# chahuja/mix-stage

Hardware: AMD Instinct MI355X
Metric: train-step clips/sec (B=32, T=64, M=8) (higher is better)
Workload: dtype f32; 1 GPU; Mix-StAGE GAN train step (reference D/G coin flip, seed 4321: 457 G + 510 D steps), B=32 clips per GPU, T=64, 128-mel, 104-dim pose, M=S=8, audio branch pinned; fp32 arithmetic (the reference trains in fp64, trainer.py:138; held to it at 1e-4 pose L1); global_batch=32, parallelism=dp1, hip_graphs=True, bn_sync=local

## Files before the change

### include/mixstage_aux.h

```cpp
#ifndef MIXSTAGE_AUX_H_
#define MIXSTAGE_AUX_H_

#include "mixstage.h"

#ifdef __cplusplus
extern "C" {
#endif

int ms_set_counter_buffer(int32_t* zeroed_counters, int n);

int ms_conv_block_bwd_overlap(const ms_conv_desc* d, const float* x, const float* x2, const float* w,
                              const float* gamma, const float* running_mean, const float* running_var,
                              const float* y_raw, const float* y, const float* save, const float* dy, float* dyr,
                              float* dx, float* dx2, float* dw, float* dbias, float* dgamma, float* dbeta,
                              void* workspace, size_t workspace_bytes, void* stream, void* side_stream,
                              void* side_workspace, size_t side_workspace_bytes);

int ms_timing_enable(int on);
size_t ms_timing_report(char* buf, size_t cap);

int ms_debug_set_patch_min_workgroups(int n);
int ms_debug_set_patch_tuning(int intra_split, int force_splitk);

int ms_debug_set_conv16_tile(int wm, int wn);
int ms_debug_set_conv16_ring(int nstg, int wide8);
int ms_debug_set_wgrad16_target(int workgroups);
int ms_debug_set_wgrad16_ring(int buffers);
int ms_debug_set_wgrad_target(int workgroups);
int ms_debug_set_wgrad_wave(int on);
int ms_debug_set_conv_tile(int on);
int ms_debug_set_bn_fused(int on);
int ms_debug_set_bn_fused_min_workgroups(int n);
int ms_debug_set_skip(const char* patterns);

int ms_debug_set_clip32(int on);

int ms_debug_set_clip_corun(int on);
int ms_debug_set_clip_corun_bwd(int on);

int ms_selftest_mfma(const float* A, const float* B, float* C, int K, void* stream);
int ms_probe_peak(int kind, long iters, void* a, void* b, double* work, void* stream);

#ifdef __cplusplus
}
#endif
#endif
```

### mix_stage_amd/_lib.py

```python
import ctypes
import os

_HERE = os.path.dirname(os.path.abspath(__file__))
LIB_PATH = os.path.join(_HERE, 'libmixstage_hip.so')
_ALT_LIB = os.environ.get('MS_LIB_PATH')
if _ALT_LIB:
  LIB_PATH = _ALT_LIB

c_void_p, c_int, c_float, c_size_t = ctypes.c_void_p, ctypes.c_int, ctypes.c_float, ctypes.c_size_t


class BwdOptions(ctypes.Structure):
  _fields_ = [('side_stream', ctypes.c_void_p), ('side_workspace', ctypes.c_void_p), ('side_workspace_bytes', ctypes.c_size_t),
              ('wt_prepared', ctypes.c_void_p), ('wgrad_partials', ctypes.c_void_p), ('defer_wgrad_launch', ctypes.c_int),
              ('prev_y', ctypes.c_void_p), ('prev_y_raw', ctypes.c_void_p), ('prev_save', ctypes.c_void_p), ('prev_gamma', ctypes.c_void_p),
              ('prev_dgamma', ctypes.c_void_p), ('prev_dbeta', ctypes.c_void_p), ('prev_dbias', ctypes.c_void_p), ('prev_slope', ctypes.c_float),
              ('bn_sync', ctypes.c_void_p), ('bn_sync_words', ctypes.c_int32), ('dy_is_dyr', ctypes.c_int),
              ('dx_accum', ctypes.c_void_p)]


class LossScale(ctypes.Structure):
  _fields_ = [('scale', ctypes.c_float), ('scale_dev', ctypes.c_void_p)]


class FwdOptions(ctypes.Structure):
  _fields_ = [('w_planes', ctypes.c_void_p), ('bn_sync', ctypes.c_void_p), ('bn_sync_words', ctypes.c_int32)]


class ConvDesc(ctypes.Structure):
  _fields_ = [(n, ctypes.c_int32) for n in
              ('B', 'Cin', 'H', 'W', 'Cout', 'groups', 'KH', 'KW', 'SH', 'SW', 'PH', 'PW', 'OH', 'OW',
               'mode', 'in_mode')] + \
             [('slope', c_float), ('eps', c_float), ('momentum', c_float), ('dtype', ctypes.c_int32)]


class ChainDesc(ctypes.Structure):
  _fields_ = [(n, ctypes.c_int32) for n in ('B', 'M', 'T', 'cin0', 'C', 'P', 'n_blocks', 'mode', 'dtype', 'sync_first_word', 'keep_all_raw')] + \
             [('slope', c_float), ('eps', c_float), ('momentum', c_float)]


class ChainTensors(ctypes.Structure):
  _fields_ = [('x', ctypes.c_void_p), ('score', ctypes.c_void_p)] + \
             [(n, ctypes.c_void_p * 4) for n in ('w', 'bias', 'gamma', 'beta', 'running_mean', 'running_var', 'y_raw', 'y', 'save')] + \
             [(n, ctypes.c_void_p) for n in ('w_logits', 'bias_logits', 'z', 'soft', 'out', 'prepared', 'sync')] + \
             [('sync_words', ctypes.c_int32)]


class Prep16Item(ctypes.Structure):
  _fields_ = [('desc', ctypes.POINTER(ConvDesc))] + [(n, ctypes.c_void_p) for n in
             ('w', 'bias', 'gamma', 'beta', 'running_mean', 'running_var', 'fwd', 'dgrad')]


MS_BARE, MS_LRELU, MS_BN_TRAIN, MS_BN_EVAL = 0, 1, 2, 3
MS_DT_BN_FROZEN = 0x800
MS_IN_PLAIN, MS_IN_BCAST, MS_IN_UP2ADD = 0, 1, 2
MS_F32, MS_BF16, MS_F16, MS_DT_OUT_F32, MS_DT_BN_FOLDED = 0, 1, 2, 0x100, 0x200
MS_DT_STAT_PAIR = 0x400

_P = c_void_p
_DESC = ctypes.POINTER(ConvDesc)

SIGNATURES = {
    'ms_last_error': (ctypes.c_char_p, []),
    'ms_abi_version': (c_int, []),
    'ms_set_counter_buffer': (c_int, [_P, c_int]),
    'ms_set_bn_sync_buffer': (c_int, [_P, c_int]),
    'ms_debug_set_bn_fused': (c_int, [c_int]),
    'ms_debug_set_bn_fused_min_workgroups': (c_int, [c_int]),
    'ms_conv_block_fwd_workspace': (c_size_t, [_DESC]),
    'ms_conv_block_bwd_workspace': (c_size_t, [_DESC]),
    'ms_conv_block_fwd': (c_int, [_DESC] + [_P] * 11 + [_P, c_size_t, _P]),
    'ms_conv_block_bwd': (c_int, [_DESC] + [_P] * 17 + [_P, c_size_t, _P]),
    'ms_conv_block_bwd_overlap': (c_int, [_DESC] + [_P] * 17 + [_P, c_size_t, _P, _P, _P, c_size_t]),
    'ms_conv_block_bwd_ex': (c_int, [_DESC] + [_P] * 17 + [_P, c_size_t, _P, _P]),
    'ms_dgrad_weights_elems': (c_size_t, [_DESC, _P]),
    'ms_dgrad_weights_prepare': (c_int, [c_int, _P, _P, _P, _P]),
    'ms_tuning_epoch': (c_int, []),
    'ms_conv_block_fwd_ex': (c_int, [_DESC] + [_P] * 11 + [_P, c_size_t, _P, _P]),
    'ms_fwd_weights_bytes': (c_size_t, [_DESC]),
    'ms_fwd_weights_prepare': (c_int, [c_int, _P, _P, _P, _P]),
    'ms_set_precision': (c_int, [c_int]),
    'ms_get_precision': (c_int, []),
    'ms_wgrad_partials_elems': (c_size_t, [_DESC, _P]),
    'ms_wgrad_reduce_multi': (c_int, [c_int, _P, _P, _P, _P, _P]),
    'ms_wgrad_flush': (c_int, [_P]),
    'ms_wgrad_discard': (c_int, []),
    'ms_weights16_bytes': (c_size_t, [_DESC, c_int]),
    'ms_weights16_prepare': (c_int, [c_int, _P, _P]),
    'ms_cb8_from_plain': (c_int, [c_int, _P, _P, c_int, c_int, c_int, _P]),
    'ms_cb8_to_plain': (c_int, [c_int, _P, _P, c_int, c_int, c_int, _P]),
    'ms_cb8_from_btc': (c_int, [c_int, _P, _P, c_int, c_int, c_int, c_int, _P]),
    'ms_cb8_to_btc': (c_int, [c_int, _P, _P, c_int, c_int, c_int, c_int, _P]),
    'ms_bn_stats': (c_int, [_P, _P, c_int, c_int, c_int, _P]),
    'ms_bn_train_apply': (c_int, [_P, c_int, c_int, _P, _P, _P, _P, _P, _P, _P, c_int, c_int, c_int, c_float, c_float, c_float, _P]),
    'ms_bn_bwd_workspace': (c_size_t, [c_int, c_int]),
    'ms_bn_bwd_sums': (c_int, [_P, _P, _P, _P, c_int, c_int, c_int, c_float, _P, c_size_t, _P]),
    'ms_bn_bwd_apply': (c_int, [_P, _P, _P, _P, _P, ctypes.c_double, _P, c_int, c_int, c_int, c_float, _P]),
    'ms_lerp_time_fwd': (c_int, [_P, _P, c_int, c_int, c_int, c_int, c_int, _P]),
    'ms_lerp_time_bwd': (c_int, [_P, _P, c_int, c_int, c_int, c_int, c_int, _P]),
    'ms_softmax_mix_fwd': (c_int, [_P, _P, _P, _P, c_int, c_int, c_int, c_int, _P]),
    'ms_softmax_mix_bwd': (c_int, [_P, _P, _P, _P, _P, c_int, c_int, c_int, c_int, _P]),
    'ms_kmeans_labels': (c_int, [_P, _P, _P, _P, c_int, c_int, c_int, c_int, c_int, c_int, _P]),
    'ms_znorm_select': (c_int, [_P, _P, _P, _P, _P, c_size_t, c_int, c_int, _P]),
    'ms_step_metrics': (c_int, [_P] * 7 + [c_int, _P, c_int, c_int, c_int, c_int, _P]),
    'ms_eval_accumulate': (c_int, [_P] * 8 + [c_int, c_int, c_int, c_int, ctypes.c_double, c_int, _P]),
    'ms_concat_style_fwd': (c_int, [_P, _P, _P, c_int, c_int, _P, c_int, c_int, c_int, c_int, _P]),
    'ms_concat_style_bwd': (c_int, [_P, _P, c_int, c_int, _P, _P, c_int, c_int, c_int, c_int, c_int, _P]),
    'ms_concat_style_soft_fwd': (c_int, [_P, _P, _P, c_int, c_int, _P, c_int, c_int, c_int, c_int, c_int, _P]),
    'ms_concat_style_soft_bwd': (c_int, [_P, _P, _P, c_int, c_int, _P, _P, _P, c_int, c_int, c_int, c_int, c_int, _P]),
    'ms_cross_entropy_fwd': (c_int, [_P, _P, _P, _P] + [c_int] * 6 + [_P]),
    'ms_cross_entropy_bwd': (c_int, [_P, _P, _P, _P] + [c_int] * 7 + [_P]),
    'ms_cross_entropy_fwd_ex': (c_int, [_P, _P, _P] + [c_int] * 6 + [_P, _P]),
    'ms_cross_entropy_bwd_ex': (c_int, [_P, _P, _P, _P] + [c_int] * 7 + [_P, _P]),
    'ms_lp_mean_fwd_ex': (c_int, [c_int, _P, _P, c_float, _P, _P, c_size_t, _P, _P]),
    'ms_lp_mean_bwd_ex': (c_int, [c_int, _P, _P, c_float, _P, _P, c_size_t, _P, _P]),
    'ms_lp_mean_pair_fwd': (c_int, [c_int, _P, _P, _P, c_size_t, _P, _P]),
    'ms_lp_mean_pair_bwd': (c_int, [c_int, _P, _P, _P, _P, _P, c_size_t, _P, _P]),
    'ms_velocity_fwd': (c_int, [_P, _P, c_int, c_int, c_int, _P]),
    'ms_velocity_bwd': (c_int, [_P, _P, c_int, c_int, c_int, _P]),
    'ms_transpose_btc': (c_int, [_P, _P, c_int, c_int, c_int, _P]),
    'ms_transpose_bct': (c_int, [_P, _P, c_int, c_int, c_int, _P]),
    'ms_l1_mean_fwd': (c_int, [_P, _P, c_float, _P, _P, c_size_t, _P]),
    'ms_l1_mean_bwd': (c_int, [_P, _P, c_float, _P, _P, c_size_t, _P]),
    'ms_l2_mean_fwd': (c_int, [_P, _P, c_float, _P, _P, c_size_t, _P]),
    'ms_l2_mean_bwd': (c_int, [_P, _P, c_float, _P, _P, c_size_t, _P]),
    'ms_copy_multi': (c_int, [c_int, _P, _P, _P, _P]),
    'ms_write_floats': (c_int, [_P, _P, c_int, _P]),
    'ms_decoder_chain_supported': (c_int, [_P]),
    'ms_decoder_chain_prepared_bytes': (c_size_t, [_P]),
    'ms_decoder_chain_workspace': (c_size_t, [_P]),
    'ms_decoder_chain_sync_words': (c_int, [_P]),
    'ms_decoder_chain_prepare': (c_int, [_P, _P, _P, _P, _P]),
    'ms_decoder_chain_fwd': (c_int, [_P, _P, _P, c_size_t, _P]),
    'ms_decoder_chain_eval_supported': (c_int, [_P]),
    'ms_decoder_chain_eval_workspace': (c_size_t, [_P]),
    'ms_decoder_chain_eval_sync_words': (c_int, [_P]),
    'ms_decoder_chain_eval_plan': (c_int, [_P, _P, _P, _P, _P, _P, c_int]),
    'ms_decoder_chain_eval_fwd': (c_int, [_P, _P, _P, c_size_t, _P]),
    'ms_sqnorm': (c_int, [_P, c_size_t, _P, _P, _P]),
    'ms_adam_step': (c_int, [_P, _P, _P, _P, c_size_t, _P, c_float, c_float, c_float, c_float, c_float, _P, _P]),
    'ms_adam_step_segmented': (c_int, [_P, _P, _P, _P, c_size_t, _P, c_float, c_float, c_float, c_float, c_float, _P, _P, _P, _P,
                                       c_int, _P]),
    'ms_adam_step_segmented_scaled': (c_int, [_P, _P, _P, _P, c_size_t, _P, c_float, c_float, c_float, c_float, c_float, _P, _P, _P, _P,
                                              c_int, _P, ctypes.c_int32, c_float, c_float, _P, c_int, _P]),
    'ms_adam_step_segmented_lr': (c_int, [_P, _P, _P, _P, c_size_t, _P, c_float, _P, c_float, c_float, c_float, _P, _P, _P, _P,
                                          c_int, _P]),
    'ms_adam_step_segmented_scaled_lr': (c_int, [_P, _P, _P, _P, c_size_t, _P, c_float, _P, c_float, c_float, c_float, _P, _P, _P, _P,
                                                 c_int, _P, ctypes.c_int32, c_float, c_float, _P, c_int, _P]),
    'ms_adam_step_segmented_ema': (c_int, [_P, _P, _P, _P, c_size_t, _P, c_float, c_float, _P, c_float, c_float, c_float, _P, _P, _P, _P,
                                           c_int, _P, ctypes.c_int32, c_float, c_float, _P, c_int, _P, c_float, _P]),
    'ms_reduce_partials_count': (c_size_t, [c_size_t]),
    'ms_timing_enable': (c_int, [c_int]),
    'ms_timing_report': (c_size_t, [ctypes.c_char_p, c_size_t]),
    'ms_debug_set_patch_min_workgroups': (c_int, [c_int]),
    'ms_debug_set_patch_tuning': (c_int, [c_int, c_int]),
    'ms_debug_set_conv16_tile': (c_int, [c_int, c_int]),
    'ms_debug_set_conv16_ring': (c_int, [c_int, c_int]),
    'ms_debug_set_skip': (c_int, [ctypes.c_char_p]),
    'ms_debug_set_clip32': (c_int, [c_int]),
    'ms_debug_set_clip_corun': (c_int, [c_int]),
    'ms_clip_hold': (c_int, [_P]),
    'ms_clip_hold_flush': (c_int, [_P]),
    'ms_clip_hold_discard': (c_int, [_P]),
    'ms_clip_grid': (c_int, [_DESC]),
    'ms_clip_pair_ok': (c_int, [_DESC, _DESC]),
    'ms_clip_dgrad_grid': (c_int, [_DESC]),
    'ms_clip_dgrad_pair_ok': (c_int, [_DESC, _DESC]),
    'ms_debug_set_clip_corun_bwd': (c_int, [c_int]),
    'ms_debug_set_wgrad16_target': (c_int, [c_int]),
    'ms_debug_set_wgrad16_ring': (c_int, [c_int]),
    'ms_debug_set_wgrad_target': (c_int, [c_int]),
    'ms_debug_set_wgrad_wave': (c_int, [c_int]),
    'ms_debug_set_conv_tile': (c_int, [c_int]),
    'ms_set_wgrad_batched': (c_int, [c_int, c_int]),
    'ms_dgrad_fuses_prev_bn': (c_int, [_P]),
    'ms_dgrad_takes_accum': (c_int, [_P]),
    'ms_stat_pair_ok': (c_int, [_P]),
    'ms_selftest_mfma': (c_int, [_P, _P, _P, c_int, _P]),
    'ms_probe_peak': (c_int, [c_int, ctypes.c_long, _P, _P, ctypes.POINTER(ctypes.c_double), _P]),
}

_lib = None


class MixStageLibError(RuntimeError):
  pass


def lib():
  global _lib
  if _lib is None:
    if not os.path.isfile(LIB_PATH):
      raise MixStageLibError('%s not built: run `make -C mix_stage_amd/csrc` (or __graft_entry__.build()); '
                             'there is no CPU fallback' % LIB_PATH)
    handle = ctypes.CDLL(LIB_PATH)
    for name, (res, args) in SIGNATURES.items():
      if _ALT_LIB and name.startswith('ms_debug_') and not hasattr(handle, name):
        continue
      fn = getattr(handle, name)
      fn.restype, fn.argtypes = res, args
    mode = os.environ.get('MS_PRECISION', '')
    if mode:
      if mode not in ('fp32', 'bf16x6'):
        raise MixStageLibError('MS_PRECISION=%s: expected fp32 or bf16x6' % mode)
      handle.ms_set_precision(1 if mode == 'bf16x6' else 0)
    if os.environ.get('MS_BN_FUSED'):
      handle.ms_debug_set_bn_fused(int(os.environ['MS_BN_FUSED']))
    if os.environ.get('MS_BN_FUSED_MIN_WGS'):
      handle.ms_debug_set_bn_fused_min_workgroups(int(os.environ['MS_BN_FUSED_MIN_WGS']))
    if os.environ.get('MS_CLIP32'):
      handle.ms_debug_set_clip32(int(os.environ['MS_CLIP32']))
    if os.environ.get('MS_CONV_TILE'):
      handle.ms_debug_set_conv_tile(int(os.environ['MS_CONV_TILE']))
    if os.environ.get('MS_WGRAD_WAVE'):
      handle.ms_debug_set_wgrad_wave(int(os.environ['MS_WGRAD_WAVE']))
    if os.environ.get('MS_PATCH_MIN_WGS'):
      handle.ms_debug_set_patch_min_workgroups(int(os.environ['MS_PATCH_MIN_WGS']))
    _lib = handle
  return _lib


def check(rc, what):
  if rc != 0:
    raise MixStageLibError('%s failed: %s' % (what, lib().ms_last_error().decode()))
```

### mix_stage_amd/csrc/conv_tile.hip

```cpp
#include <algorithm>
#include <cstdint>

#include "kernels.h"

#ifndef MS_TILE_OCC
#define MS_TILE_OCC 3
#endif
namespace ms {

int g_conv_tile = 1;

template <int KH, int KW>
struct TileCfg {
  static constexpr int KHW = KH * KW;
  static constexpr int CK = KHW == 4 ? 8 : KHW == 9 ? 4 : KHW == 16 ? 2 : KHW == 24 ? 2 : 4;
  static constexpr int KSTEP = CK * KHW;
};

constexpr int tile_row_pitch(int win, int sv, int tw) {
  int rp = win;
  if (tw >= 32) return rp;
  while ((rp * sv) % 32 != 16) rp += 4;
  return rp;
}

template <int KH, int KW, int S, int TW, int AM, int WM, int WN>
__global__ __launch_bounds__(256, (KH * KW == 16 || KH * KW == 4 || (AM == 1 && WM == 1)) ? MS_TILE_OCC : 2) void conv_tile_kernel(const PatchArgs p) {
  prefetch_kernargs<sizeof(PatchArgs)>();
  using Cfg = TileCfg<KH, KW>;
  static_assert(WM * WN == 4, "four waves");
  constexpr int BM = 64 * WM, BN = 64 * WN, TH = BN / TW;
  constexpr int SV = S;
  constexpr int CK = Cfg::CK, KHW = Cfg::KHW, KSTEP = Cfg::KSTEP;
  constexpr int PR = (TH - 1) * SV + KH;
  constexpr int WIN = ((TW - 1) * S + KW + 3 + 3) / 4 * 4, W4 = WIN / 4;
  constexpr int RP = tile_row_pitch(WIN, SV, TW), CP = PR * RP;
  constexpr int KH2 = KSTEP / 2;
  constexpr int AP = KSTEP % 8 == 4 ? KSTEP : KSTEP + 4;
  constexpr int ABUF = BM * AP;
  constexpr int STAGE = ABUF + CK * CP + 16;
  static_assert(CK % 2 == 0 && (AP / 4) % 2 == 1 && AP >= KSTEP, "bad weight-slice pitch");
  constexpr int NB4 = CK * PR * W4, NB = (NB4 + 255) / 256;
  constexpr int NAV = BM * (KSTEP / 4), NA = (NAV + 255) / 256;
  constexpr int RUN4 = BM * KHW / 4;
  static_assert(KSTEP % 4 == 0 && BN % TW == 0 && (BM * KHW) % 4 == 0 && (KSTEP / 2) % 2 == 0, "bad tile configuration");
  static_assert(2 * STAGE >= 2 * WN * BM + 64, "statistics exchange does not fit the staging buffers");
  __shared__ __attribute__((aligned(16))) float smem[2 * STAGE];

  const int t = threadIdx.x, lane = t & 63, khalf = lane >> 5, l31 = lane & 31;
  const int wid = __builtin_amdgcn_readfirstlane(t >> 6);
  const int wm = wid / WN, wn = wid - wm * WN;
  const int vid = xcd_remap(blockIdx.x, p.gx * p.gy * p.gz);
  const int cls_f = (p.ncls > 1 && p.cls_fast) ? vid % p.ncls : 0;
  const int vid2 = (p.ncls > 1 && p.cls_fast) ? vid / p.ncls : vid;
  const int by_ = vid2 % p.gy, bx_ = (vid2 / p.gy) % p.gx, bz_ = vid2 / (p.gy * p.gx);
  const int zz = p.groups * p.splitk;
  const int cls = (p.ncls > 1 && !p.cls_fast) ? bz_ / zz : cls_f, bzc = (p.ncls > 1 && !p.cls_fast) ? bz_ - cls * zz : bz_;
  const int g = bzc / p.splitk, ks = bzc - g * p.splitk, m0 = by_ * BM;
  const int PHc = p.ncls > 1 ? p.cls_PH[cls] : p.PH, PWc = p.ncls > 1 ? p.cls_PW[cls] : p.PW;
  const int OUTHc = p.ncls > 1 ? p.cls_OUTH[cls] : p.OUTH, OUTWc = p.ncls > 1 ? p.cls_OUTW[cls] : p.OUTW;
  const int o_ryc = p.ncls > 1 ? p.cls_ry[cls] : p.o_ry, o_rxc = p.ncls > 1 ? p.cls_rx[cls] : p.o_rx;
  const int tiles_per_img = p.tiles_y * p.tiles_x;
  const int img = bx_ / tiles_per_img;
  const int trem = bx_ - img * tiles_per_img;
  const int tyi = trem / p.tiles_x, txi = trem - tyi * p.tiles_x;
  const int oy0 = tyi * TH, ox0 = txi * TW;
  const int PWA = (PWc + 3) & ~3, shift = PWA - PWc;
  const int iy0 = oy0 * SV - PHc, ix0 = ox0 * S - PWA;
  const int cbase = p.bcast ? 0 : g * p.Kc;
  const int Kg = p.Kg;

  unsigned goff[NB];
  int loff[NB], gci[NB];
#pragma unroll
  for (int i = 0; i < NB; ++i) {
    const int e = t + i * 256;
    const int ci = e / (PR * W4), rem = e - ci * (PR * W4), r = rem / W4, f = rem - r * W4;
    const int iy = iy0 + r, ix = ix0 + 4 * f;
    const bool ok = (e < NB4) & ((unsigned)iy < (unsigned)p.SRCH) & ((unsigned)ix < (unsigned)p.SRCW);
    goff[i] = ok ? 4u * (unsigned)(ci * p.s_chan + iy * p.s_row + ix) : BUF_OOB;
    gci[i] = ci;
    loff[i] = e < NB4 ? ci * CP + r * RP + 4 * f : CK * CP;
  }
  unsigned aoff[NA];
  int lsto[AM == 2 ? NA : 1][4];
#pragma unroll
  for (int i = 0; i < NA; ++i) {
    const int idx = t + i * 256;
    if (AM == 2) {
      const int co = idx / RUN4, q4 = idx - co * RUN4;
      aoff[i] = idx < NAV ? 4u * (unsigned)((co * p.Mg + m0) * KHW + 4 * q4) : BUF_OOB;
#pragma unroll
      for (int j = 0; j < 4; ++j) {
        const int e = 4 * q4 + j, cil = e / KHW, tap = e - cil * KHW;
        lsto[i][j] = idx < NAV ? cil * AP + co * KHW + (KHW - 1 - tap) : ABUF + CK * CP + 4 + j;
      }
    } else {
      const int row = idx / (KSTEP / 4), kq = idx - row * (KSTEP / 4);
      aoff[i] = (idx < NAV && m0 + row < p.Mg) ? 4u * (unsigned)((m0 + row) * Kg + kq * 4) : BUF_OOB;
    }
  }
  const __amdgpu_buffer_rsrc_t rsA = buf_rsrc(p.A), rsS = buf_rsrc(p.src);
  const unsigned a_group = (unsigned)cls * p.cls_a_stride + (unsigned)g * p.Mg * Kg;
  const int img_base = img * p.s_img;

  float4 raa[1][NA], rbb[1][NB];
  auto load_chunk = [&](int ci0, const int set) {
    float4 (&ra)[NA] = raa[0];
    float4 (&rb)[NB] = rbb[0];
    (void)set;
    const int k0 = ci0 * KHW;
    const unsigned sa = __builtin_amdgcn_readfirstlane(AM == 2 ? 4u * (a_group + (unsigned)(ci0 * p.Mg * KHW)) : 4u * (a_group + (unsigned)k0));
    const bool full_k = k0 + KSTEP <= Kg;
#pragma unroll
    for (int i = 0; i < NA; ++i) {
      if (AM == 2) {
        const int co = (t + i * 256) / RUN4;
        ra[i] = buf_load4(rsA, (full_k | (ci0 + co < p.Kc)) ? aoff[i] : BUF_OOB, sa);
      } else {
        const int kq = (t + i * 256) % (KSTEP / 4);
        ra[i] = buf_load4(rsA, (full_k | (k0 + kq * 4 < Kg)) ? aoff[i] : BUF_OOB, sa);
      }
    }
    const unsigned cb = __builtin_amdgcn_readfirstlane(4u * (unsigned)(img_base + (cbase + ci0) * p.s_chan));
    const bool full_c = ci0 + CK <= p.Kc;
#pragma unroll
    for (int i = 0; i < NB; ++i) rb[i] = buf_load4(rsS, (full_c | (ci0 + gci[i] < p.Kc)) ? goff[i] : BUF_OOB, cb);
  };
  auto store_chunk = [&](int buf, const int set) {
    const float4 (&ra)[NA] = raa[0];
    const float4 (&rb)[NB] = rbb[0];
    (void)set;
    float* As = smem + buf * STAGE;
    float* Ps = As + ABUF;
#pragma unroll
    for (int i = 0; i < NA; ++i) {
      if (AM == 2) {
        As[lsto[i][0]] = ra[i].x; As[lsto[i][1]] = ra[i].y; As[lsto[i][2]] = ra[i].z; As[lsto[i][3]] = ra[i].w;
      } else {
        const int idx = t + i * 256;
        const int row = idx / (KSTEP / 4), kq = idx - row * (KSTEP / 4);
        *reinterpret_cast<float4*>(As + (idx < NAV ? row * AP + 4 * kq : ABUF + CK * CP + 8)) = ra[i];
      }
    }
#pragma unroll
    for (int i = 0; i < NB; ++i) *reinterpret_cast<float4*>(Ps + loff[i]) = rb[i];
  };

  f32x16 acc[2][2];
#pragma unroll
  for (int mi = 0; mi < 2; ++mi)
#pragma unroll
    for (int ni = 0; ni < 2; ++ni)
#pragma unroll
      for (int r = 0; r < 16; ++r) acc[mi][ni][r] = 0.f;

  const int a_base = (64 * wm + l31) * AP + khalf * KH2;
  int b_base[2];
#pragma unroll
  for (int ni = 0; ni < 2; ++ni) {
    const int nloc = 64 * wn + 32 * ni + l31;
    const int ty = nloc / TW, tx = nloc - ty * TW;
    b_base[ni] = ty * SV * RP + tx * S + shift + khalf * (CK / 2) * CP;
  }

  const int chunk_beg = ks * p.chunks_per_split;
  const int nchunks = min((p.Kc + CK - 1) / CK - chunk_beg, p.chunks_per_split);
  auto compute_chunk = [&](int cur) {
    const float* As = smem + cur * STAGE;
    const float* Ps = As + ABUF;
    constexpr int NG = (KH2 + 3) / 4;
    float av[2][2][4], bv[2][4][2];
    auto read_group = [&](int gi, int slot) {
      const int kk0 = 4 * gi;
      constexpr int dummy = 0; (void)dummy;
#pragma unroll
      for (int mi = 0; mi < 2; ++mi) {
        if (kk0 + 4 <= KH2) {
          const float4 v = *reinterpret_cast<const float4*>(As + a_base + 32 * mi * AP + kk0);
          av[slot][mi][0] = v.x; av[slot][mi][1] = v.y; av[slot][mi][2] = v.z; av[slot][mi][3] = v.w;
        } else {
          const float2 v = *reinterpret_cast<const float2*>(As + a_base + 32 * mi * AP + kk0);
          av[slot][mi][0] = v.x; av[slot][mi][1] = v.y;
        }
      }
#pragma unroll
      for (int r = 0; r < 4; ++r) {
        const int kk = kk0 + r;
        if (kk < KH2) {
          const int ci = kk / KHW, rr = kk - ci * KHW, kh = rr / KW, kw = rr - kh * KW;
          const int offb = ci * CP + kh * RP + kw;
#pragma unroll
          for (int ni = 0; ni < 2; ++ni) bv[slot][r][ni] = Ps[b_base[ni] + offb];
        }
      }
    };
    read_group(0, 0);
#pragma unroll
    for (int gi = 0; gi < NG; ++gi) {
      if (gi + 1 < NG) read_group(gi + 1, (gi + 1) & 1);
      __builtin_amdgcn_sched_barrier(0);
#pragma unroll
      for (int r = 0; r < 4; ++r)
        if (4 * gi + r < KH2) {
#pragma unroll
          for (int mi = 0; mi < 2; ++mi)
#pragma unroll
            for (int ni = 0; ni < 2; ++ni)
              acc[mi][ni] = __builtin_amdgcn_mfma_f32_32x32x2f32(av[gi & 1][mi][r], bv[gi & 1][r][ni], acc[mi][ni], 0, 0, 0);
        }
      __builtin_amdgcn_sched_barrier(0);
    }
  };
  if (nchunks > 0) {
    load_chunk(chunk_beg * CK, 0);
    store_chunk(0, 0);
    if (nchunks > 1) load_chunk((chunk_beg + 1) * CK, 0);
  }
  __syncthreads();
  for (int ch = 0; ch < nchunks; ch += 2) {
    if (ch + 1 < nchunks) store_chunk(1, 0);
    if (ch + 2 < nchunks) load_chunk((chunk_beg + ch + 2) * CK, 0);
    compute_chunk(0);
    __syncthreads();
    if (ch + 1 >= nchunks) break;
    if (ch + 2 < nchunks) store_chunk(0, 0);
    if (ch + 3 < nchunks) load_chunk((chunk_beg + ch + 3) * CK, 0);
    compute_chunk(1);
    __syncthreads();
  }

  const int ctot = p.groups * p.Mg;
  const int ep = p.ep;
  int ooff[2];
  bool cval[2];
#pragma unroll
  for (int ni = 0; ni < 2; ++ni) {
    const int nloc = 64 * wn + 32 * ni + l31;
    const int oy = oy0 + nloc / TW, ox = ox0 + nloc % TW;
    cval[ni] = (oy < OUTHc) & (ox < OUTWc);
    ooff[ni] = img * p.o_img + (oy * p.o_sh + o_ryc) * p.o_row + ox * p.o_sw + o_rxc;
  }
  if (p.part) {
    float* part = p.part + (size_t)ks * p.part_stride;
#pragma unroll
    for (int mi = 0; mi < 2; ++mi)
#pragma unroll
      for (int ni = 0; ni < 2; ++ni)
#pragma unroll
        for (int r = 0; r < 16; ++r) {
          const int m = m0 + 64 * wm + 32 * mi + (r & 3) + 8 * (r >> 2) + 4 * khalf;
          if (m < p.Mg && cval[ni]) part[(size_t)ooff[ni] + (size_t)(g * p.Mg + m) * p.o_chan] = acc[mi][ni][r];
        }
    return;
  }
  const bool stats = ep == EP_RAW_STATS;
  int cnt_w = 0;
  if (stats) {
    const int ty_lo = (64 * wn) / TW, ty_hi = (64 * wn + 63) / TW;
    const int cols = min(TW, OUTWc - ox0);
    cnt_w = max(0, min(ty_hi + 1, OUTHc - oy0) - ty_lo) * max(0, cols);
  }
  const float inv_cnt = cnt_w > 0 ? 1.0f / (float)cnt_w : 0.f;
  float keep_s = 0.f, keep_m2 = 0.f;
#pragma unroll
  for (int mi = 0; mi < 2; ++mi) {
    float sc_r[16], sh_r[16];
#pragma unroll
    for (int r = 0; r < 16; ++r) {
      const int m = m0 + 64 * wm + 32 * mi + (r & 3) + 8 * (r >> 2) + 4 * khalf;
      const int chn = g * p.Mg + (m < p.Mg ? m : 0);
      const float bsv = p.bias ? p.bias[chn] : 0.f;
      if (ep == EP_BN_EVAL) {
        const float inv = 1.0f / sqrtf(p.bn_v[chn] + p.eps);
        sc_r[r] = p.bn_g[chn] * inv;
        sh_r[r] = fmaf(bsv - p.bn_m[chn], sc_r[r], p.bn_b[chn]);
      } else {
        sc_r[r] = 1.f; sh_r[r] = bsv;
      }
    }
#pragma unroll
    for (int r = 0; r < 16; ++r) {
      const int m = m0 + 64 * wm + 32 * mi + (r & 3) + 8 * (r >> 2) + 4 * khalf;
      const bool mval = m < p.Mg;
      const int chn = g * p.Mg + (mval ? m : 0);
      float v[2], srow = 0.f;
#pragma unroll
      for (int ni = 0; ni < 2; ++ni) {
        v[ni] = ep == EP_BN_EVAL ? fmaf(acc[mi][ni][r], sc_r[r], sh_r[r]) : acc[mi][ni][r] + sh_r[r];
        if (stats) srow += cval[ni] ? v[ni] : 0.f;
        float o = v[ni];
        if (ep == EP_BN_EVAL || ep == EP_LRELU) o = lrelu(o, p.slope);
        if (mval && cval[ni]) p.out[(size_t)ooff[ni] + (size_t)chn * p.o_chan] = o;
      }
      if (stats) {
        const float sw = half_wave_sum(srow);
        const float mean = sw * inv_cnt;
        float q = 0.f;
#pragma unroll
        for (int ni = 0; ni < 2; ++ni) {
          const float dlt = v[ni] - mean;
          q += cval[ni] ? dlt * dlt : 0.f;
        }
        const float m2w = half_wave_sum(q);
        if (l31 == 16 * mi + r) { keep_s = sw; keep_m2 = m2w; }
      }
    }
  }

  if (stats) {
    float* red = smem;
    __syncthreads();
    {
      const int mi = l31 >> 4, r = l31 & 15;
      const int ml = 64 * wm + 32 * mi + (r & 3) + 8 * (r >> 2) + 4 * khalf;
      red[(wn * BM + ml) * 2 + 0] = keep_s;
      red[(wn * BM + ml) * 2 + 1] = keep_m2;
    }
    int* cnts = reinterpret_cast<int*>(red + 2 * WN * BM);
    if (lane == 0 && wm == 0) cnts[wn] = cnt_w;
    __syncthreads();
    if (t < BM && m0 + t < p.Mg) {
      float n_a = 0.f, s_a = 0.f, m2_a = 0.f;
#pragma unroll
      for (int w = 0; w < WN; ++w) {
        const float n_b = (float)cnts[w];
        if (n_b > 0.f) {
          const float s_b = red[(w * BM + t) * 2], m2_b = red[(w * BM + t) * 2 + 1];
          if (n_a == 0.f) { n_a = n_b; s_a = s_b; m2_a = m2_b; }
          else {
            const float dlt = s_b / n_b - s_a / n_a;
            m2_a = m2_a + m2_b + dlt * dlt * (n_a * n_b / (n_a + n_b));
            s_a += s_b; n_a += n_b;
          }
        }
      }
      float* st = p.stats + ((size_t)bx_ * ctot + g * p.Mg + m0 + t) * 2;
      st[0] = s_a;
      st[1] = m2_a;
      if (t == 0 && by_ == 0 && g == 0) p.counts[bx_] = n_a;
    }
  }
}

bool conv_tile_shape_ok(int KH, int KW, int S) {
  return (KH == 3 && KW == 3 && S == 1) || (KH == 4 && KW == 4 && S == 2) || (KH == 2 && KW == 2 && S == 1) || (KH == 3 && KW == 8 && S == 1);
}

template <int KH, int KW, int S, int AM>
static void launch_tile_tw(const PatchArgs& a, int tw, int wide, dim3 grid, hipStream_t s) {
#define MS_TK(TW, WM, WN) hipLaunchKernelGGL((conv_tile_kernel<KH, KW, S, TW, AM, WM, WN>), grid, dim3(256), 0, s, a)
  if (wide) { if (tw == 32) MS_TK(32, 1, 4); else MS_TK(16, 1, 4); }
  else { if (tw == 32) MS_TK(32, 2, 2); else MS_TK(16, 2, 2); }
#undef MS_TK
}

int launch_tile(const PatchArgs& a, const PatchPlan& pl, int KH, int KW, int S, double flops, double bytes, hipStream_t s) {
  const int wide = pl.tile == 2 ? 1 : 0;
  const int bm = wide ? 64 : 128;
  PatchArgs b = a;
  if (a.ncls > 4) return set_error("tile conv: more than 4 parity classes");
  b.gx = pl.n_tiles; b.gy = cdiv(a.Mg, bm); b.gz = a.groups * a.splitk * std::max(1, a.ncls);
  { static int cf = -1; if (cf < 0) { const char* e = getenv("MS_CLS_FAST"); cf = e ? atoi(e) : 1; } b.cls_fast = cf; }
  if ((double)b.gx * b.gy * b.gz > 2.0e9) return set_error("conv grid too large");
  dim3 grid(b.gx * b.gy * b.gz);
  if (a.splitk < 1 || (a.splitk > 1 && !a.part)) return set_error("tile conv: bad split-K setup");
  if (a.src_elems >= (1u << 29) || a.a_elems >= (1u << 29)) return set_error("tile conv: operand of 2 GiB or more");
  const int am = a.a_vec == 2 ? 2 : 1;
  if (am == 2 && a.Mg % bm) return set_error("tile conv: in-place weights need whole channel tiles");
  TimingScope ts(s, flops, bytes, "conv_tile_kernel<%d,%d,%d,%d,%d,%d>|conv_%s_tile k%dx%d s%d Mg%d Kg%d g%d tiles%d tile%dx%d tw%d splitk%d%s",
                 KH, KW, S, pl.tw, am, wide, a.is_dgrad ? "dgrad" : "fwd", KH, KW, S, a.Mg, a.Kg, a.groups, pl.n_tiles, bm, wide ? 256 : 128,
                 pl.tw, a.splitk, (a.ep == EP_RAW_STATS && !a.part) ? " +bnstats" : "");
  if (ts.skip()) return 0;
  if (am == 2) {
    if (KH == 3 && KW == 3) launch_tile_tw<3, 3, 1, 2>(b, pl.tw, wide, grid, s);
    else if (KH == 3 && KW == 8) launch_tile_tw<3, 8, 1, 2>(b, pl.tw, wide, grid, s);
    else return set_error("tile conv: no in-place instance for this shape");
  } else {
    if (KH == 3 && KW == 3) launch_tile_tw<3, 3, 1, 1>(b, pl.tw, wide, grid, s);
    else if (KH == 4 && KW == 4) launch_tile_tw<4, 4, 2, 1>(b, pl.tw, wide, grid, s);
    else if (KH == 2 && KW == 2) launch_tile_tw<2, 2, 1, 1>(b, pl.tw, wide, grid, s);
    else launch_tile_tw<3, 8, 1, 1>(b, pl.tw, wide, grid, s);
  }
  return check_launch("conv_tile_kernel");
}

}

extern "C" int ms_debug_set_conv_tile(int on) {
  const int old = ms::g_conv_tile;
  if (old != (on ? 1 : 0)) ms_debug_set_patch_min_workgroups(ms::g_patch_min_wgs);
  ms::g_conv_tile = on ? 1 : 0;
  return old;
}
```

Baseline: 11440 clips/s.

## Interleave next-chunk global loads and LDS stores into MFMA loop of tile conv

Adds a PIPE variant of the tile convolution kernel that breaks the staging of the next K-chunk into per-item global loads and LDS stores, then issues them between MFMA groups using sched_barrier fences. The goal is to hide global-memory and LDS-store latency behind matrix math instead of running them in bulk before each compute phase. Out-of-range chunks are masked through zero limits, so the loop needs fewer branches. By default the variant is used only for selected shape/tile combinations, and a debug switch plus an environment variable control it. Spreading loads across the loop keeps more registers live and could lower occupancy or upset the compiler's scheduling.

```diff
diff --git a/include/mixstage_aux.h b/include/mixstage_aux.h
--- a/include/mixstage_aux.h
+++ b/include/mixstage_aux.h
@@ -29,6 +29,7 @@
 int ms_debug_set_wgrad_target(int workgroups);
 int ms_debug_set_wgrad_wave(int on);
 int ms_debug_set_conv_tile(int on);
+int ms_debug_set_tile_pipeline(int on);
 int ms_debug_set_bn_fused(int on);
 int ms_debug_set_bn_fused_min_workgroups(int n);
 int ms_debug_set_skip(const char* patterns);
diff --git a/mix_stage_amd/_lib.py b/mix_stage_amd/_lib.py
--- a/mix_stage_amd/_lib.py
+++ b/mix_stage_amd/_lib.py
@@ -172,6 +172,7 @@
     'ms_debug_set_wgrad_target': (c_int, [c_int]),
     'ms_debug_set_wgrad_wave': (c_int, [c_int]),
     'ms_debug_set_conv_tile': (c_int, [c_int]),
+    'ms_debug_set_tile_pipeline': (c_int, [c_int]),
     'ms_set_wgrad_batched': (c_int, [c_int, c_int]),
     'ms_dgrad_fuses_prev_bn': (c_int, [_P]),
     'ms_dgrad_takes_accum': (c_int, [_P]),
@@ -212,6 +213,8 @@
       handle.ms_debug_set_clip32(int(os.environ['MS_CLIP32']))
     if os.environ.get('MS_CONV_TILE'):
       handle.ms_debug_set_conv_tile(int(os.environ['MS_CONV_TILE']))
+    if os.environ.get('MS_TILE_PIPE') and hasattr(handle, 'ms_debug_set_tile_pipeline'):
+      handle.ms_debug_set_tile_pipeline(int(os.environ['MS_TILE_PIPE']))
     if os.environ.get('MS_WGRAD_WAVE'):
       handle.ms_debug_set_wgrad_wave(int(os.environ['MS_WGRAD_WAVE']))
     if os.environ.get('MS_PATCH_MIN_WGS'):
diff --git a/mix_stage_amd/csrc/conv_tile.hip b/mix_stage_amd/csrc/conv_tile.hip
--- a/mix_stage_amd/csrc/conv_tile.hip
+++ b/mix_stage_amd/csrc/conv_tile.hip
@@ -9,6 +9,7 @@
 namespace ms {
 
 int g_conv_tile = 1;
+int g_tile_pipe = 1;
 
 template <int KH, int KW>
 struct TileCfg {
@@ -24,7 +25,7 @@
   return rp;
 }
 
-template <int KH, int KW, int S, int TW, int AM, int WM, int WN>
+template <int KH, int KW, int S, int TW, int AM, int WM, int WN, bool PIPE>
 __global__ __launch_bounds__(256, (KH * KW == 16 || KH * KW == 4 || (AM == 1 && WM == 1)) ? MS_TILE_OCC : 2) void conv_tile_kernel(const PatchArgs p) {
   prefetch_kernargs<sizeof(PatchArgs)>();
   using Cfg = TileCfg<KH, KW>;
@@ -104,37 +105,38 @@
   const unsigned a_group = (unsigned)cls * p.cls_a_stride + (unsigned)g * p.Mg * Kg;
   const int img_base = img * p.s_img;
 
-  float4 raa[1][NA], rbb[1][NB];
-  auto load_chunk = [&](int ci0, const int set) {
-    float4 (&ra)[NA] = raa[0];
-    float4 (&rb)[NB] = rbb[0];
-    (void)set;
-    const int k0 = ci0 * KHW;
-    const unsigned sa = __builtin_amdgcn_readfirstlane(AM == 2 ? 4u * (a_group + (unsigned)(ci0 * p.Mg * KHW)) : 4u * (a_group + (unsigned)k0));
-    const bool full_k = k0 + KSTEP <= Kg;
-#pragma unroll
-    for (int i = 0; i < NA; ++i) {
+  float4 ra[NA], rb[NB];
+  constexpr int NIT = NA + NB;
+  struct ChunkSrc { int ci0, k0, klim, clim; unsigned sa, cb; bool full_k, full_c; };
+  auto chunk_src = [&](int ci0, bool live) {
+    ChunkSrc c;
+    c.ci0 = ci0; c.k0 = ci0 * KHW; c.klim = live ? Kg : 0; c.clim = live ? p.Kc : 0;
+    c.sa = __builtin_amdgcn_readfirstlane(AM == 2 ? 4u * (a_group + (unsigned)(ci0 * p.Mg * KHW)) : 4u * (a_group + (unsigned)c.k0));
+    c.cb = __builtin_amdgcn_readfirstlane(4u * (unsigned)(img_base + (cbase + ci0) * p.s_chan));
+    c.full_k = c.k0 + KSTEP <= c.klim;
+    c.full_c = ci0 + CK <= c.clim;
+    return c;
+  };
+  auto load_item = [&](const int it, const ChunkSrc& c) {
+    if (it < NA) {
+      const int i = it;
       if (AM == 2) {
         const int co = (t + i * 256) / RUN4;
-        ra[i] = buf_load4(rsA, (full_k | (ci0 + co < p.Kc)) ? aoff[i] : BUF_OOB, sa);
+        ra[i] = buf_load4(rsA, (c.full_k | (c.ci0 + co < c.clim)) ? aoff[i] : BUF_OOB, c.sa);
       } else {
         const int kq = (t + i * 256) % (KSTEP / 4);
-        ra[i] = buf_load4(rsA, (full_k | (k0 + kq * 4 < Kg)) ? aoff[i] : BUF_OOB, sa);
-      }
-    }
-    const unsigned cb = __builtin_amdgcn_readfirstlane(4u * (unsigned)(img_base + (cbase + ci0) * p.s_chan));
-    const bool full_c = ci0 + CK <= p.Kc;
-#pragma unroll
-    for (int i = 0; i < NB; ++i) rb[i] = buf_load4(rsS, (full_c | (ci0 + gci[i] < p.Kc)) ? goff[i] : BUF_OOB, cb);
-  };
-  auto store_chunk = [&](int buf, const int set) {
-    const float4 (&ra)[NA] = raa[0];
-    const float4 (&rb)[NB] = rbb[0];
-    (void)set;
+        ra[i] = buf_load4(rsA, (c.full_k | (c.k0 + kq * 4 < c.klim)) ? aoff[i] : BUF_OOB, c.sa);
+      }
+    } else {
+      const int i = it - NA;
+      rb[i] = buf_load4(rsS, (c.full_c | (c.ci0 + gci[i] < c.clim)) ? goff[i] : BUF_OOB, c.cb);
+    }
+  };
+  auto store_item = [&](const int it, int buf) {
     float* As = smem + buf * STAGE;
     float* Ps = As + ABUF;
-#pragma unroll
-    for (int i = 0; i < NA; ++i) {
+    if (it < NA) {
+      const int i = it;
       if (AM == 2) {
         As[lsto[i][0]] = ra[i].x; As[lsto[i][1]] = ra[i].y; As[lsto[i][2]] = ra[i].z; As[lsto[i][3]] = ra[i].w;
       } else {
@@ -142,9 +144,18 @@
         const int row = idx / (KSTEP / 4), kq = idx - row * (KSTEP / 4);
         *reinterpret_cast<float4*>(As + (idx < NAV ? row * AP + 4 * kq : ABUF + CK * CP + 8)) = ra[i];
       }
-    }
-#pragma unroll
-    for (int i = 0; i < NB; ++i) *reinterpret_cast<float4*>(Ps + loff[i]) = rb[i];
+    } else {
+      *reinterpret_cast<float4*>(Ps + loff[it - NA]) = rb[it - NA];
+    }
+  };
+  auto load_chunk = [&](int ci0, bool live) {
+    const ChunkSrc c = chunk_src(ci0, live);
+#pragma unroll
+    for (int it = 0; it < NIT; ++it) load_item(it, c);
+  };
+  auto store_chunk = [&](int buf) {
+#pragma unroll
+    for (int it = 0; it < NIT; ++it) store_item(it, buf);
   };
 
   f32x16 acc[2][2];
@@ -166,7 +177,9 @@
 
   const int chunk_beg = ks * p.chunks_per_split;
   const int nchunks = min((p.Kc + CK - 1) / CK - chunk_beg, p.chunks_per_split);
-  auto compute_chunk = [&](int cur) {
+  constexpr int ISTR = KH2 / NIT;
+  static_assert(!PIPE || ISTR >= 1, "more staging items than MFMA slots");
+  auto compute_chunk = [&](int cur, auto&& stage) {
     const float* As = smem + cur * STAGE;
     const float* Ps = As + ABUF;
     constexpr int NG = (KH2 + 3) / 4;
@@ -208,26 +221,52 @@
 #pragma unroll
             for (int ni = 0; ni < 2; ++ni)
               acc[mi][ni] = __builtin_amdgcn_mfma_f32_32x32x2f32(av[gi & 1][mi][r], bv[gi & 1][r][ni], acc[mi][ni], 0, 0, 0);
+          if (PIPE && (4 * gi + r) % ISTR == 0 && (4 * gi + r) / ISTR < NIT) {
+            __builtin_amdgcn_sched_barrier(0);
+            stage((4 * gi + r) / ISTR);
+            __builtin_amdgcn_sched_barrier(0);
+          }
         }
       __builtin_amdgcn_sched_barrier(0);
     }
   };
-  if (nchunks > 0) {
-    load_chunk(chunk_beg * CK, 0);
-    store_chunk(0, 0);
-    if (nchunks > 1) load_chunk((chunk_beg + 1) * CK, 0);
-  }
-  __syncthreads();
-  for (int ch = 0; ch < nchunks; ch += 2) {
-    if (ch + 1 < nchunks) store_chunk(1, 0);
-    if (ch + 2 < nchunks) load_chunk((chunk_beg + ch + 2) * CK, 0);
-    compute_chunk(0);
+  if constexpr (PIPE) {
+    load_chunk(chunk_beg * CK, nchunks > 0);
+    store_chunk(0);
+    load_chunk((chunk_beg + 1) * CK, nchunks > 1);
     __syncthreads();
-    if (ch + 1 >= nchunks) break;
-    if (ch + 2 < nchunks) store_chunk(0, 0);
-    if (ch + 3 < nchunks) load_chunk((chunk_beg + ch + 3) * CK, 0);
-    compute_chunk(1);
+    int ch = 0;
+    for (; ch + 1 < nchunks; ch += 2) {
+      const ChunkSrc c2 = chunk_src((chunk_beg + ch + 2) * CK, ch + 2 < nchunks);
+      compute_chunk(0, [&](const int it) { store_item(it, 1); __builtin_amdgcn_sched_barrier(0); load_item(it, c2); });
+      __syncthreads();
+      const ChunkSrc c3 = chunk_src((chunk_beg + ch + 3) * CK, ch + 3 < nchunks);
+      compute_chunk(1, [&](const int it) { store_item(it, 0); __builtin_amdgcn_sched_barrier(0); load_item(it, c3); });
+      __syncthreads();
+    }
+    if (ch < nchunks) {
+      compute_chunk(0, [](const int) {});
+      __syncthreads();
+    }
+  } else {
+    auto none = [](const int) {};
+    if (nchunks > 0) {
+      load_chunk(chunk_beg * CK, true);
+      store_chunk(0);
+      if (nchunks > 1) load_chunk((chunk_beg + 1) * CK, true);
+    }
     __syncthreads();
+    for (int ch = 0; ch < nchunks; ch += 2) {
+      if (ch + 1 < nchunks) store_chunk(1);
+      if (ch + 2 < nchunks) load_chunk((chunk_beg + ch + 2) * CK, true);
+      compute_chunk(0, none);
+      __syncthreads();
+      if (ch + 1 >= nchunks) break;
+      if (ch + 2 < nchunks) store_chunk(0);
+      if (ch + 3 < nchunks) load_chunk((chunk_beg + ch + 3) * CK, true);
+      compute_chunk(1, none);
+      __syncthreads();
+    }
   }
 
   const int ctot = p.groups * p.Mg;
@@ -347,9 +386,26 @@
   return (KH == 3 && KW == 3 && S == 1) || (KH == 4 && KW == 4 && S == 2) || (KH == 2 && KW == 2 && S == 1) || (KH == 3 && KW == 8 && S == 1);
 }
 
+static bool tile_pipe_default(int KH, int KW, int tw, int am, int wide) {
+  if (KH == 2 && KW == 2) return !wide;
+  if (KH == 3 && KW == 3) return tw == 32 && ((am == 1 && !wide) || (am == 2 && wide));
+  if (KH == 4 && KW == 4) return tw == 32 && wide;
+  return false;
+}
+
+constexpr bool tile_pipe_fits(int KH, int KW, int AM, int WM) {
+  return !(KH == 3 && KW == 3 && AM == 1 && WM == 1) && !(KH == 3 && KW == 8 && AM == 2 && WM == 1);
+}
+
 template <int KH, int KW, int S, int AM>
-static void launch_tile_tw(const PatchArgs& a, int tw, int wide, dim3 grid, hipStream_t s) {
-#define MS_TK(TW, WM, WN) hipLaunchKernelGGL((conv_tile_kernel<KH, KW, S, TW, AM, WM, WN>), grid, dim3(256), 0, s, a)
+static void launch_tile_tw(const PatchArgs& a, int tw, int wide, bool pipe, dim3 grid, hipStream_t s) {
+#define MS_TK(TW, WM, WN)                                                                                              \
+  do {                                                                                                                 \
+    if constexpr (tile_pipe_fits(KH, KW, AM, WM)) {                                                                    \
+      if (pipe) { hipLaunchKernelGGL((conv_tile_kernel<KH, KW, S, TW, AM, WM, WN, true>), grid, dim3(256), 0, s, a); break; } \
+    }                                                                                                                  \
+    hipLaunchKernelGGL((conv_tile_kernel<KH, KW, S, TW, AM, WM, WN, false>), grid, dim3(256), 0, s, a);                \
+  } while (0)
   if (wide) { if (tw == 32) MS_TK(32, 1, 4); else MS_TK(16, 1, 4); }
   else { if (tw == 32) MS_TK(32, 2, 2); else MS_TK(16, 2, 2); }
 #undef MS_TK
@@ -372,15 +428,16 @@
                  KH, KW, S, pl.tw, am, wide, a.is_dgrad ? "dgrad" : "fwd", KH, KW, S, a.Mg, a.Kg, a.groups, pl.n_tiles, bm, wide ? 256 : 128,
                  pl.tw, a.splitk, (a.ep == EP_RAW_STATS && !a.part) ? " +bnstats" : "");
   if (ts.skip()) return 0;
+  const bool pipe = g_tile_pipe >= 2 || (g_tile_pipe == 1 && tile_pipe_default(KH, KW, pl.tw, am, wide));
   if (am == 2) {
-    if (KH == 3 && KW == 3) launch_tile_tw<3, 3, 1, 2>(b, pl.tw, wide, grid, s);
-    else if (KH == 3 && KW == 8) launch_tile_tw<3, 8, 1, 2>(b, pl.tw, wide, grid, s);
+    if (KH == 3 && KW == 3) launch_tile_tw<3, 3, 1, 2>(b, pl.tw, wide, pipe, grid, s);
+    else if (KH == 3 && KW == 8) launch_tile_tw<3, 8, 1, 2>(b, pl.tw, wide, pipe, grid, s);
     else return set_error("tile conv: no in-place instance for this shape");
   } else {
-    if (KH == 3 && KW == 3) launch_tile_tw<3, 3, 1, 1>(b, pl.tw, wide, grid, s);
-    else if (KH == 4 && KW == 4) launch_tile_tw<4, 4, 2, 1>(b, pl.tw, wide, grid, s);
-    else if (KH == 2 && KW == 2) launch_tile_tw<2, 2, 1, 1>(b, pl.tw, wide, grid, s);
-    else launch_tile_tw<3, 8, 1, 1>(b, pl.tw, wide, grid, s);
+    if (KH == 3 && KW == 3) launch_tile_tw<3, 3, 1, 1>(b, pl.tw, wide, pipe, grid, s);
+    else if (KH == 4 && KW == 4) launch_tile_tw<4, 4, 2, 1>(b, pl.tw, wide, pipe, grid, s);
+    else if (KH == 2 && KW == 2) launch_tile_tw<2, 2, 1, 1>(b, pl.tw, wide, pipe, grid, s);
+    else launch_tile_tw<3, 8, 1, 1>(b, pl.tw, wide, pipe, grid, s);
   }
   return check_launch("conv_tile_kernel");
 }
@@ -393,3 +450,9 @@
   ms::g_conv_tile = on ? 1 : 0;
   return old;
 }
+
+extern "C" int ms_debug_set_tile_pipeline(int on) {
+  const int old = ms::g_tile_pipe;
+  ms::g_tile_pipe = on < 0 ? 0 : on > 2 ? 2 : on;
+  return old;
+}
```

Result: no change. 11530 clips/s, median of 6 (+0.8%).
